# mihikamd/DP-GSAT

Hardware: AMD Instinct MI355X
Metric: million edges/s (attn+sample+aggregate fwd+bwd) (higher is better)
Workload: dtype f32

## Files before the change

dp_gsat_amd/csrc/common.h:

```cpp
#pragma once
#include <cstring>
#include <cstdint>
#include <cstdio>
#include <cstdarg>
#include <hip/hip_runtime.h>

#include "../../include/gsat_hip.h"

namespace gsat {

void set_error(const char* fmt, ...);
const char* get_error();

#define GSAT_CHECK_HIP(expr)                                                                  \
    do {                                                                                      \
        hipError_t _e = (expr);                                                               \
        if (_e != hipSuccess) {                                                               \
            gsat::set_error("%s:%d: %s -> %s", __FILE__, __LINE__, #expr, hipGetErrorString(_e)); \
            return GSAT_ERR_HIP;                                                              \
        }                                                                                     \
    } while (0)

#define GSAT_REQUIRE(cond, code, ...)                                                         \
    do {                                                                                      \
        if (!(cond)) {                                                                        \
            gsat::set_error(__VA_ARGS__);                                                     \
            return (code);                                                                    \
        }                                                                                     \
    } while (0)

#define GSAT_LAUNCH_CHECK() GSAT_CHECK_HIP(hipGetLastError())

static inline int64_t ceil_div(int64_t a, int64_t b) { return (a + b - 1) / b; }

hipError_t zero_async(void* p, size_t bytes, hipStream_t stream);
static inline size_t align_up(size_t a, size_t b) { return (a + b - 1) / b * b; }

struct Arena {
    char* base;
    size_t cap, off;
    Arena(void* p, size_t bytes) : base(static_cast<char*>(p)), cap(bytes), off(0) {}
    template <class T> T* take(size_t n) {
        size_t b = align_up(n * sizeof(T), 256);
        if (base == nullptr || off + b > cap) { off += b; return nullptr; }
        T* r = reinterpret_cast<T*>(base + off);
        off += b;
        return r;
    }
    bool ok() const { return base != nullptr && off <= cap; }
};

struct SlabJob { const float* ws; int nslab; size_t slab; int M, N; int64_t ldc; int accumulate; float* out; };
int gemm_f32(hipStream_t stream, bool a_t, bool b_t, int64_t M, int64_t N, int64_t K, const float* A, int64_t lda, const float* B,
             int64_t ldb, float* C, int64_t ldc, const float* bias, bool accumulate, float* ws, size_t ws_floats, bool allow_split = false,
             SlabJob* defer = nullptr);
int slab_reduce_jobs(hipStream_t stream, const SlabJob* jobs, int n);
size_t gemm_workspace_floats(int64_t M, int64_t N, int64_t K, bool reduce_rows);
struct WgradPlan { int eligible, S, rows; size_t ws_floats; };
WgradPlan wgrad_plan(int64_t Mo, int64_t No, int64_t K);
size_t gemm_wgrad_workspace_floats(int64_t Mo, int64_t No, int64_t K);
int gemm_wgrad(hipStream_t stream, int64_t Mo, int64_t No, int64_t K, const float* A, int64_t lda, const float* B, int64_t ldb, float* C,
               int64_t ldc, bool accumulate, float* ws, size_t ws_floats, SlabJob* defer = nullptr);

int aggr_sum_fwd_impl(hipStream_t stream, const float* x, const float* self_rows, const float* att, const float* edge_emb,
                      const int32_t* rowptr, const int32_t* col, const int32_t* eid, int64_t N, int64_t E, int64_t H, float self_coef,
                      float* out, const int32_t* chunk_ptr, float* partial);

#ifdef __HIPCC__
constexpr int WAVE = 64;

template <int CTRL> __device__ __forceinline__ float dpp_add(float v) {
    const int t = __builtin_amdgcn_update_dpp(0, __builtin_bit_cast(int, v), CTRL, 0xF, 0xF, true);
    return v + __builtin_bit_cast(float, t);
}

template <int WIDTH> __device__ __forceinline__ float group_sum(float v) {
    if constexpr ((WIDTH & (WIDTH - 1)) == 0) {
        if constexpr (WIDTH >= 2) v = dpp_add<0xB1>(v);
        if constexpr (WIDTH >= 4) v = dpp_add<0x4E>(v);
        if constexpr (WIDTH >= 8) v = dpp_add<0x141>(v);
        if constexpr (WIDTH >= 16) v = dpp_add<0x140>(v);
        if constexpr (WIDTH >= 32) v += __builtin_bit_cast(float, __builtin_amdgcn_ds_swizzle(__builtin_bit_cast(int, v), 0x401F));
        if constexpr (WIDTH >= 64) v += __shfl_xor(v, 32, 64);
    } else {
        const int l = (int)(threadIdx.x & 63) % WIDTH;
#pragma unroll
        for (int o = 16; o > 0; o >>= 1) {
            const float t = __shfl_down(v, o, 64);
            if (l + o < WIDTH) v += t;
        }
    }
    return v;
}

template <int LPR, int BLOCK> struct LaneGroups {
    static constexpr int GPW = 64 / LPR, GPB = (BLOCK / 64) * GPW;
    int grp, lane;
    __device__ __forceinline__ LaneGroups() {
        const int wl = threadIdx.x & 63, sub = wl / LPR;
        lane = wl % LPR;
        grp = sub < GPW ? (int)(threadIdx.x >> 6) * GPW + sub : -1;
    }
};

__device__ __forceinline__ float4 ld4(const float* p) { return *reinterpret_cast<const float4*>(p); }
__device__ __forceinline__ void st4(float* p, float4 v) { *reinterpret_cast<float4*>(p) = v; }
__device__ __forceinline__ void st4_nt(float* p, float4 v) {
    typedef float v4f __attribute__((ext_vector_type(4)));
    v4f t = {v.x, v.y, v.z, v.w};
    __builtin_nontemporal_store(t, reinterpret_cast<v4f*>(p));
}
__device__ __forceinline__ float4 ld4_off(const float* base, uint32_t byte_off) {
    return *reinterpret_cast<const float4*>(reinterpret_cast<const char*>(base) + byte_off);
}
__device__ __forceinline__ void st4_off(float* base, uint32_t byte_off, float4 v) {
    *reinterpret_cast<float4*>(reinterpret_cast<char*>(base) + byte_off) = v;
}
__device__ __forceinline__ void st4_lds(float4* p, float4 v) {
    typedef float v4f __attribute__((ext_vector_type(4)));
    v4f t = {v.x, v.y, v.z, v.w};
    *(__attribute__((address_space(3))) v4f*)p = t;
}
__device__ __forceinline__ void st1_lds(float* p, float v) { *(__attribute__((address_space(3))) float*)p = v; }
__device__ __forceinline__ float4 f4zero() { return make_float4(0.f, 0.f, 0.f, 0.f); }
__device__ __forceinline__ float4 f4fma(float a, float4 x, float4 acc) {
    acc.x = fmaf(a, x.x, acc.x); acc.y = fmaf(a, x.y, acc.y);
    acc.z = fmaf(a, x.z, acc.z); acc.w = fmaf(a, x.w, acc.w);
    return acc;
}
__device__ __forceinline__ float f4dot(float4 a, float4 b) {
    return fmaf(a.x, b.x, fmaf(a.y, b.y, fmaf(a.z, b.z, a.w * b.w)));
}

__device__ __forceinline__ uint4 philox4x32(uint64_t seed, uint32_t c0, uint32_t c1, uint32_t c2, uint32_t c3) {
    uint32_t k0 = (uint32_t)seed, k1 = (uint32_t)(seed >> 32);
#pragma unroll
    for (int r = 0; r < 10; ++r) {
        uint64_t p0 = (uint64_t)0xD2511F53u * c0;
        uint64_t p1 = (uint64_t)0xCD9E8D57u * c2;
        uint32_t n0 = (uint32_t)(p1 >> 32) ^ c1 ^ k0;
        uint32_t n1 = (uint32_t)p1;
        uint32_t n2 = (uint32_t)(p0 >> 32) ^ c3 ^ k1;
        uint32_t n3 = (uint32_t)p0;
        c0 = n0; c1 = n1; c2 = n2; c3 = n3;
        k0 += 0x9E3779B9u; k1 += 0xBB67AE85u;
    }
    return make_uint4(c0, c1, c2, c3);
}

__device__ __forceinline__ float philox_noise_u(uint64_t seed, int row) {
    const uint4 r = philox4x32(seed, (uint32_t)row, 0u, 4u, 0x5A17u);
    return ((float)(r.x >> 9) + 0.5f) * (1.0f / 8388608.0f);
}

struct SeedRef {
    uint64_t value;
    const uint64_t* dev;
    __device__ __forceinline__ uint64_t get() const { return dev ? *dev : value; }
};

__device__ __forceinline__ float4 philox_keep4(uint64_t seed, int layer, int row, int c, float p) {
    uint4 r = philox4x32(seed, (uint32_t)row, (uint32_t)(c >> 2), (uint32_t)layer, 0x5A17u);
    const float k = 1.0f / 16777216.0f;
    return make_float4((float)(r.x >> 8) * k >= p ? 1.f : 0.f, (float)(r.y >> 8) * k >= p ? 1.f : 0.f,
                       (float)(r.z >> 8) * k >= p ? 1.f : 0.f, (float)(r.w >> 8) * k >= p ? 1.f : 0.f);
}
#endif

}
```

dp_gsat_amd/csrc/pna.hip:

```cpp
#include "common.h"
#include "pna_math.h"

namespace gsat {

constexpr int PNA_BLOCK = 128;
constexpr int SC_AMP = GSAT_SCALE_AMPLIFICATION, SC_ATT = GSAT_SCALE_ATTENUATION, SC_LIN = GSAT_SCALE_LINEAR, SC_INVLIN = GSAT_SCALE_INVERSE_LINEAR;

struct PnaCfg {
    int A, S;
    int aggr[8];
    int scal[8];
    float avg_lin, avg_log;
};

__device__ __forceinline__ int pna_xcd_remap(int b, int nb) {
    int q = nb >> 3, r = nb & 7, x = b & 7, i = b >> 3;
    return (x < r ? x * (q + 1) : r * (q + 1) + (x - r) * q) + i;
}

__device__ __forceinline__ float scaler_factor(int s, float deg, float avg_lin, float avg_log) {
    switch (s) {
        case SC_AMP: return logf(deg + 1.f) / avg_log;
        case SC_ATT: return deg == 0.f ? 1.f : avg_log / logf(deg + 1.f);
        case SC_LIN: return deg / avg_lin;
// ... 420 lines not shown
                        aj.add(m);
                        if (HAS_EE) {
                            float4 me = f4scale(w[u], ev[u]);
                            if (me.x < ae.mn.x) emin.x = kk; if (me.y < ae.mn.y) emin.y = kk; if (me.z < ae.mn.z) emin.z = kk; if (me.w < ae.mn.w) emin.w = kk;
                            if (me.x > ae.mx.x) emax.x = kk; if (me.y > ae.mx.y) emax.y = kk; if (me.z > ae.mx.z) emax.z = kk; if (me.w > ae.mx.w) emax.w = kk;
                            ae.add(me);
                        }
                    }
                }
            }
        }
        const Acc4 ai = self_stats(xi, sa, sa2, amin, amax);
        float t1 = 0.f, t2 = 0.f, tmn = 0.f, tmx = 0.f;
        float4 Pi = f4zero(), Qi = f4zero(), Pj = f4zero(), Qj = f4zero(), Pe = f4zero(), Qe = f4zero();
        float4 gmn_i = f4zero(), gmx_i = f4zero(), gmn_j = f4zero(), gmx_j = f4zero(), gmn_e = f4zero(), gmx_e = f4zero();
        if (on) {
            const float n = fmaxf(cnt, 1.f), inv_n = 1.f / n;
            const float* drow = dout + (size_t)row * out_stride + c;
            if (staged) asm volatile("s_waitcnt vmcnt(0)" ::: "memory");
#define GSAT_FOLD(ACC, PART, P, Q, GMN, GMX)                                                                           \
            {                                                                                                          \
                const float4 mean = f4scale(inv_n, ACC.s);                                                             \
                float4 var = make_float4(ACC.q.x * inv_n - mean.x * mean.x, ACC.q.y * inv_n - mean.y * mean.y,         \
                                         ACC.q.z * inv_n - mean.z * mean.z, ACC.q.w * inv_n - mean.w * mean.w);        \
                const float4 hs = make_float4(var.x > 0.f ? 0.5f / sqrtf(var.x + 1e-5f) : 0.f, var.y > 0.f ? 0.5f / sqrtf(var.y + 1e-5f) : 0.f, \
                                              var.z > 0.f ? 0.5f / sqrtf(var.z + 1e-5f) : 0.f, var.w > 0.f ? 0.5f / sqrtf(var.w + 1e-5f) : 0.f); \
                float4 p0 = f4zero(), gv = f4zero();                                                                   \
                if (NAGG) {                                                                                            \
                    p0 = f4scale(inv_n, stage[0 * parts + (PART)][threadIdx.x]);                                       \
                    if (NAGG == 5) { const float4 vsum = stage[4 * parts + (PART)][threadIdx.x];                       \
                                     p0 = make_float4(p0.x + vsum.x, p0.y + vsum.y, p0.z + vsum.z, p0.w + vsum.w); }   \
                    GMN = stage[1 * parts + (PART)][threadIdx.x];                                                      \
                    GMX = stage[2 * parts + (PART)][threadIdx.x];                                                      \
                    const float4 vs = stage[3 * parts + (PART)][threadIdx.x];                                          \
                    gv = make_float4(vs.x * hs.x, vs.y * hs.y, vs.z * hs.z, vs.w * hs.w);                              \
                } else                                                                                                 \
                for (int s = 0; s < cfg.S; ++s) {                                                                      \
                    const float f = scaler_factor(cfg.scal[s], cnt, cfg.avg_lin, cfg.avg_log);                         \
                    for (int a = 0; a < cfg.A; ++a) {                                                                  \
                        const int sg_ = (s * cfg.A + a) * parts + (PART);                                              \
                        const float4 v = f4scale(f, staged ? stage[sg_][threadIdx.x] : ld4(drow + (size_t)sg_ * H));   \
                        switch (cfg.aggr[a]) {                                                                         \
                            case AGG_SUM: p0.x += v.x; p0.y += v.y; p0.z += v.z; p0.w += v.w; break;                   \
                            case AGG_MEAN: p0 = f4fma(inv_n, v, p0); break;                                            \
                            case AGG_MIN: GMN.x += v.x; GMN.y += v.y; GMN.z += v.z; GMN.w += v.w; break;               \
                            case AGG_MAX: GMX.x += v.x; GMX.y += v.y; GMX.z += v.z; GMX.w += v.w; break;               \
                            case AGG_VAR: gv.x += v.x; gv.y += v.y; gv.z += v.z; gv.w += v.w; break;                   \
                            default: gv.x = fmaf(v.x, hs.x, gv.x); gv.y = fmaf(v.y, hs.y, gv.y);                       \
                                     gv.z = fmaf(v.z, hs.z, gv.z); gv.w = fmaf(v.w, hs.w, gv.w); break;                \
                        }                                                                                              \
                    }                                                                                                  \
                }                                                                                                      \
                Q = f4scale(2.f * inv_n, gv);                                                                          \
                P = make_float4(p0.x - mean.x * Q.x, p0.y - mean.y * Q.y, p0.z - mean.z * Q.z, p0.w - mean.w * Q.w);   \
            }
            GSAT_FOLD(ai, 0, Pi, Qi, gmn_i, gmx_i)
            {
#define GSAT_SELF(C)                                                                                                   \
            {                                                                                                          \
                const float xc = xi.C;                                                                                 \
                const float wlo = xc > 0.f ? amin : (xc < 0.f ? amax : wfirst), whi = xc > 0.f ? amax : (xc < 0.f ? amin : wfirst); \
                dxi.C = Pi.C * sa + Qi.C * xc * sa2 + gmn_i.C * wlo + gmx_i.C * whi;                                   \
                t1 = fmaf(Pi.C, xc, t1);                                                                               \
                t2 = fmaf(Qi.C * xc, xc, t2);                                                                          \
                tmn += xc > 0.f ? gmn_i.C * xc : (xc < 0.f ? gmx_i.C * xc : 0.f);                                      \
                tmx += xc > 0.f ? gmx_i.C * xc : (xc < 0.f ? gmn_i.C * xc : 0.f);                                      \
            }
            float4 dxi;
            GSAT_SELF(x) GSAT_SELF(y) GSAT_SELF(z) GSAT_SELF(w)
#undef GSAT_SELF
            st4(dx_self + (size_t)row * H + c, dxi);
            }
            GSAT_FOLD(aj, 1, Pj, Qj, gmn_j, gmx_j)
            if (HAS_EE) { GSAT_FOLD(ae, 2, Pe, Qe, gmn_e, gmx_e) }
#undef GSAT_FOLD
        }
        if (LONG) {
            float* r = partial + (size_t)chunk_ptr[row] * rec;
            if (on) {
                st4(r + c, Pj); st4(r + H + c, Qj); st4(r + 2 * H + c, gmn_j); st4(r + 3 * H + c, gmx_j);
                st4i(r + 4 * H + c, jmin); st4i(r + 5 * H + c, jmax);
                if (HAS_EE) {
                    float* re = r + 6 * H;
                    st4(re + c, Pe); st4(re + H + c, Qe); st4(re + 2 * H + c, gmn_e); st4(re + 3 * H + c, gmx_e);
                    st4i(re + 4 * H + c, emin); st4i(re + 5 * H + c, emax);
                }
            }
            const float s1 = group_sum<LPR>(t1), s2 = group_sum<LPR>(t2), smn = group_sum<LPR>(tmn), smx = group_sum<LPR>(tmx);
            if (lane == 0) {
                st4(r + (size_t)6 * GP * H, make_float4(s1, s2, smn, smx));
                st4(r + (size_t)6 * GP * H + 4, make_float4(__int_as_float(kmin_a), __int_as_float(kmax_a), 0.f, 0.f));
            }
            continue;
        }
        for (int kb = beg; kb < end; kb += 4) {
            const int nb = min(4, end - kb);
            int j4[4], e4[4];
            float w4[4];
            float4 x4[4], ee4[4];
            if (end - beg <= 4) {
#pragma unroll
                for (int u = 0; u < 4; ++u) { j4[u] = lj[u]; e4[u] = le[u]; w4[u] = lw[u]; }
            } else {
#pragma unroll
                for (int u = 0; u < 4; ++u) {
                    j4[u] = u < nb ? col[kb + u] : 0;
                    e4[u] = u < nb ? eid[kb + u] : 0;
                }
#pragma unroll
                for (int u = 0; u < 4; ++u) w4[u] = (u < nb && att) ? att[e4[u]] : 1.f;
            }
#pragma unroll
            for (int u = 0; u < 4; ++u) {
                x4[u] = (u < nb && on) ? ld4(x + (size_t)j4[u] * H + c) : f4zero();
                if (HAS_EE) ee4[u] = (u < nb && on) ? ld4(edge_emb + (size_t)e4[u] * H + c) : f4zero();
            }
#pragma unroll
            for (int u = 0; u < 4; ++u) {
                if (u >= nb) continue;
                const int k = kb + u, e = e4[u];
                const float w = w4[u];
                const float4 xj = x4[u];
                float da = 0.f;
                if (on) {
                    float4 dm;
                    dm.x = fmaf(Qj.x, w * xj.x, Pj.x) + (k == jmin.x ? gmn_j.x : 0.f) + (k == jmax.x ? gmx_j.x : 0.f);
                    dm.y = fmaf(Qj.y, w * xj.y, Pj.y) + (k == jmin.y ? gmn_j.y : 0.f) + (k == jmax.y ? gmx_j.y : 0.f);
                    dm.z = fmaf(Qj.z, w * xj.z, Pj.z) + (k == jmin.z ? gmn_j.z : 0.f) + (k == jmax.z ? gmx_j.z : 0.f);
                    dm.w = fmaf(Qj.w, w * xj.w, Pj.w) + (k == jmin.w ? gmn_j.w : 0.f) + (k == jmax.w ? gmx_j.w : 0.f);
                    st4(dmsg + (size_t)k * H + c, f4scale(w, dm));
                    da += f4dot(dm, xj);
                    da += t1 + w * t2 + (k == kmin_a ? tmn : 0.f) + (k == kmax_a ? tmx : 0.f);
                    if (HAS_EE) {
                        const float4 ee = ee4[u];
                        float4 de;
                        de.x = fmaf(Qe.x, w * ee.x, Pe.x) + (k == emin.x ? gmn_e.x : 0.f) + (k == emax.x ? gmx_e.x : 0.f);
                        de.y = fmaf(Qe.y, w * ee.y, Pe.y) + (k == emin.y ? gmn_e.y : 0.f) + (k == emax.y ? gmx_e.y : 0.f);
                        de.z = fmaf(Qe.z, w * ee.z, Pe.z) + (k == emin.z ? gmn_e.z : 0.f) + (k == emax.z ? gmx_e.z : 0.f);
                        de.w = fmaf(Qe.w, w * ee.w, Pe.w) + (k == emin.w ? gmn_e.w : 0.f) + (k == emax.w ? gmx_e.w : 0.f);
                        if (dedge) st4(dedge + (size_t)e * H + c, f4scale(w, de));
                        da += f4dot(de, ee);
                    }
                }
                if (datt) {
                    da = group_sum<LPR>(da);
                    if (lane == 0) datt[e] = c0 ? datt[e] + da : da;
                }
            }
        }
    }
}

constexpr int TILE_BLOCK = 512;

__global__ void k_pna_tiles(const int32_t* __restrict__ node_ptr, const int32_t* __restrict__ node_seg, const int32_t* __restrict__ rowptr,
                            const int32_t* __restrict__ rowptr_src, int N, int TN, int slack, int T, int4* __restrict__ desc,
                            int32_t* __restrict__ spill_count) {
    const int t = blockIdx.x * blockDim.x + threadIdx.x;
    if (t == 0 && spill_count) *spill_count = 0;
    if (t > T) return;
    const int64_t p = (int64_t)t * TN;
    int start = N;
    if (t < T && p < N) {
        start = (int)p;
        if (node_seg) {
            const int g0 = node_ptr[node_seg[p]];
            start = min((int)p, max(g0, (int)p - slack));
        }
    }
    desc[t] = make_int4(start, rowptr[start], rowptr_src[start], 0);
}

template <int LPR, int NAGG, bool NATT>
__global__ __launch_bounds__(TILE_BLOCK, 4) void k_pna_bwd_tile(
    const float* __restrict__ x, const float* __restrict__ att, const float* __restrict__ dout, const int32_t* __restrict__ rowptr,
    const int32_t* __restrict__ col, const int32_t* __restrict__ eid, const int4* __restrict__ desc,
    const int32_t* __restrict__ rowptr_src, const int32_t* __restrict__ slot_map, int H, int TE, int RCAP, float* dx,
    float* __restrict__ dmsg, float* datt, float* __restrict__ dw, const float* __restrict__ dx_add, int datt_acc) {
    constexpr int GPB = LaneGroups<LPR, TILE_BLOCK>::GPB;
    constexpr int RPW = 64 / LPR;
    constexpr int NSEG = NAGG * 2;
    extern __shared__ float4 smem4[];
    float4* erow = smem4;
    int* s_col = reinterpret_cast<int*>(erow + (size_t)TE * LPR);
    int* s_eid = s_col + TE;
    float* s_w = reinterpret_cast<float*>(s_eid);
    float* s_att = reinterpret_cast<float*>(s_eid + TE);
    int* s_slot = reinterpret_cast<int*>(s_att + TE);
    int* s_rp = s_slot + TE;
    int* s_rps = s_rp + RCAP + 1;
    float* s_na = reinterpret_cast<float*>(s_rps + RCAP + 1);
    float* s_dna = s_na + RCAP + 1;
    const int tid = threadIdx.x, wave = tid >> 6;
    const LaneGroups<LPR, TILE_BLOCK> lg;
    const int grp = lg.grp < 0 ? GPB : lg.grp;
    const int lane = lg.lane, c = lane * 4;
    const bool on = c < H && lg.grp >= 0;
    const int t = pna_xcd_remap(blockIdx.x, gridDim.x);
    const int4 d0 = desc[t], d1 = desc[t + 1];
    const int n0 = d0.x, n1 = d1.x;
    if (n1 <= n0) return;
    const int nr = n1 - n0;
    const int k0 = d0.y, ne = min(d1.y - k0, TE);
    const int s0 = d0.z, ns = d1.z - s0, nsl = min(ns, TE);
    float4 dcur[NSEG];
    float4 xi_cur = f4zero();
    const uint32_t hb = (uint32_t)H * 4u, gb = NSEG * hb, cb = (uint32_t)c * 4u;
    const float* gwin = dout + (size_t)n0 * NSEG * H;
    const float* xwin = x + (size_t)n0 * H;
    float* dxwin = dx + (size_t)n0 * H;
    float* mwin = dmsg + (size_t)k0 * H;
    int r = lg.grp >= 0 ? grp : nr;
#pragma unroll
    for (int sg = 0; sg < NSEG; ++sg) dcur[sg] = f4zero();
    if (r < nr && on) {
#pragma unroll
        for (int sg = 0; sg < NSEG; ++sg) dcur[sg] = ld4_off(gwin, r * gb + sg * hb + cb);
        xi_cur = ld4_off(xwin, r * hb + cb);
    }
    for (int i = tid; i <= nr; i += TILE_BLOCK) {
        s_rp[i] = rowptr[n0 + i] - k0;
        s_rps[i] = rowptr_src[n0 + i] - s0;
        if (NATT) { s_na[i] = att[min(n0 + i, n1 - 1)]; s_dna[i] = 0.f; }
    }
    for (int i = tid; i < ne; i += TILE_BLOCK) {
        s_col[i] = col[k0 + i];
        if (!NATT) s_eid[i] = eid[k0 + i];
    }
    for (int i = tid; i < nsl; i += TILE_BLOCK) s_slot[i] = slot_map[s0 + i] - k0;
    __syncthreads();
    for (int base = 0; base < ne; base += GPB) {
        const int i = base + grp;
        if (i < ne && on)
            __builtin_amdgcn_global_load_lds((const __attribute__((address_space(1))) void*)(x + (size_t)s_col[i] * H + c),
                                             (__attribute__((address_space(3))) void*)(erow + (size_t)(base + wave * RPW) * LPR), 16, 0, 0);
    }
    for (int i = tid; i < ne; i += TILE_BLOCK) {
        if (NATT) {
            s_att[i] = att[s_col[i]];
        } else {
            s_att[i] = att ? att[s_eid[i]] : 1.f;
        }
    }
    asm volatile("s_waitcnt vmcnt(0)" ::: "memory");
    __syncthreads();
    float4 dx_keep = f4zero();
    for (; r < nr; r += GPB) {
        const int nr_ = r + GPB;
        const int beg = s_rp[r], end = s_rp[r + 1];
        const float na_row = NATT ? s_na[r] : 0.f;
        const float cnt = (float)(end - beg);
        float sa = 0.f, sa2 = 0.f, amin = INFINITY, amax = -INFINITY;
        int kmin_a = beg, kmax_a = beg;
        Acc4 aj;
        aj.init();
        int4 jmin = make_int4(beg, beg, beg, beg), jmax = jmin;
        float wfirst = 1.f;
        const int mid = min(end, max(beg, ne));
        auto stats = [&](int k, float w, float4 xv) {
            if (k == beg) wfirst = w;
            sa += w; sa2 = fmaf(w, w, sa2);
            if (w < amin) { amin = w; kmin_a = k; }
            if (w > amax) { amax = w; kmax_a = k; }
            const float4 m = f4scale(w, xv);
#define GSAT_TARG(C)                                                                                                       \
            if (m.C < aj.mn.C) { jmin.C = k; aj.mn.C = m.C; }                                                              \
            if (m.C > aj.mx.C) { jmax.C = k; aj.mx.C = m.C; }
            GSAT_TARG(x) GSAT_TARG(y) GSAT_TARG(z) GSAT_TARG(w)
#undef GSAT_TARG
            aj.s.x += m.x; aj.s.y += m.y; aj.s.z += m.z; aj.s.w += m.w;
            aj.q.x = fmaf(m.x, m.x, aj.q.x); aj.q.y = fmaf(m.y, m.y, aj.q.y); aj.q.z = fmaf(m.z, m.z, aj.q.z); aj.q.w = fmaf(m.w, m.w, aj.q.w);
        };
        for (int k = beg; k < mid; ++k)
            stats(k, NATT ? s_att[k] * na_row : s_att[k], on ? erow[(size_t)k * LPR + lane] : f4zero());
        for (int k = mid; k < end; ++k)
            stats(k, NATT ? att[col[k0 + k]] * na_row : (att ? att[eid[k0 + k]] : 1.f), on ? ld4(x + (size_t)col[k0 + k] * H + c) : f4zero());
        const float4 xi = xi_cur;
        const Acc4 ai = self_stats(xi, sa, sa2, amin, amax);
        const float n = fmaxf(cnt, 1.f), inv_n = 1.f / n;
        float t1 = 0.f, t2 = 0.f, tmn = 0.f, tmx = 0.f;
        float4 Pi, Qi, Pj, Qj, gmn_i, gmx_i, gmn_j, gmx_j;
#define GSAT_TFOLD(ACC, PART, P, Q, GMN, GMX)                                                                              \
        {                                                                                                                  \
            const float4 mean = f4scale(inv_n, ACC.s);                                                                     \
            const float4 var = make_float4(ACC.q.x * inv_n - mean.x * mean.x, ACC.q.y * inv_n - mean.y * mean.y,           \
                                           ACC.q.z * inv_n - mean.z * mean.z, ACC.q.w * inv_n - mean.w * mean.w);          \
            const float4 hs = make_float4(var.x > 0.f ? 0.5f * __builtin_amdgcn_rsqf(var.x + 1e-5f) : 0.f,                 \
                                          var.y > 0.f ? 0.5f * __builtin_amdgcn_rsqf(var.y + 1e-5f) : 0.f,                 \
                                          var.z > 0.f ? 0.5f * __builtin_amdgcn_rsqf(var.z + 1e-5f) : 0.f,                 \
                                          var.w > 0.f ? 0.5f * __builtin_amdgcn_rsqf(var.w + 1e-5f) : 0.f);                \
            float4 p0 = f4scale(inv_n, dcur[0 * 2 + (PART)]);                                                              \
            if (NAGG == 5) { const float4 vsum = dcur[(NAGG == 5 ? 4 : 0) * 2 + (PART)];                                   \
                             p0 = make_float4(p0.x + vsum.x, p0.y + vsum.y, p0.z + vsum.z, p0.w + vsum.w); }               \
            GMN = dcur[1 * 2 + (PART)];                                                                                    \
            GMX = dcur[2 * 2 + (PART)];                                                                                    \
            const float4 vs = dcur[3 * 2 + (PART)];                                                                        \
            const float4 gv = make_float4(vs.x * hs.x, vs.y * hs.y, vs.z * hs.z, vs.w * hs.w);                             \
            Q = f4scale(2.f * inv_n, gv);                                                                                  \
            P = make_float4(p0.x - mean.x * Q.x, p0.y - mean.y * Q.y, p0.z - mean.z * Q.z, p0.w - mean.w * Q.w);           \
        }
        GSAT_TFOLD(ai, 0, Pi, Qi, gmn_i, gmx_i)
        if (on) {
            float4 dxi;
#define GSAT_TSELF(C)                                                                                                      \
            {                                                                                                              \
                const float xc = xi.C;                                                                                     \
                const float wlo = xc > 0.f ? amin : (xc < 0.f ? amax : wfirst), whi = xc > 0.f ? amax : (xc < 0.f ? amin : wfirst); \
                dxi.C = Pi.C * sa + Qi.C * xc * sa2 + gmn_i.C * wlo + gmx_i.C * whi;                                       \
                t1 = fmaf(Pi.C, xc, t1);                                                                                   \
                t2 = fmaf(Qi.C * xc, xc, t2);                                                                              \
                tmn += xc > 0.f ? gmn_i.C * xc : (xc < 0.f ? gmx_i.C * xc : 0.f);                                          \
                tmx += xc > 0.f ? gmx_i.C * xc : (xc < 0.f ? gmn_i.C * xc : 0.f);                                          \
            }
            GSAT_TSELF(x) GSAT_TSELF(y) GSAT_TSELF(z) GSAT_TSELF(w)
#undef GSAT_TSELF
            if (end == beg) dxi = f4zero();
            if (nr_ < nr) st4_off(dxwin, r * hb + cb, dxi); else dx_keep = dxi;
        }
        GSAT_TFOLD(aj, 1, Pj, Qj, gmn_j, gmx_j)
#undef GSAT_TFOLD
        if (nr_ < nr && on) {
#pragma unroll
            for (int sg = 0; sg < NSEG; ++sg) dcur[sg] = ld4_off(gwin, nr_ * gb + sg * hb + cb);
            xi_cur = ld4_off(xwin, nr_ * hb + cb);
        }
        float dna_acc = 0.f;
        auto grad = [&](int k, float w, float a_src, int j, int e, float4 xj, bool lds) {
            const bool in_lds = lds && j >= n0 && j < n1;
            float da = 0.f;
            if (on) {
                float4 dm;
                dm.x = fmaf(Qj.x, w * xj.x, Pj.x) + (k == jmin.x ? gmn_j.x : 0.f) + (k == jmax.x ? gmx_j.x : 0.f);
                dm.y = fmaf(Qj.y, w * xj.y, Pj.y) + (k == jmin.y ? gmn_j.y : 0.f) + (k == jmax.y ? gmx_j.y : 0.f);
                dm.z = fmaf(Qj.z, w * xj.z, Pj.z) + (k == jmin.z ? gmn_j.z : 0.f) + (k == jmax.z ? gmx_j.z : 0.f);
                dm.w = fmaf(Qj.w, w * xj.w, Pj.w) + (k == jmin.w ? gmn_j.w : 0.f) + (k == jmax.w ? gmx_j.w : 0.f);
                const float4 o = f4scale(w, dm);
                if (in_lds) st4_lds(erow + (size_t)k * LPR + lane, o);
                else if (lds) st4_off(mwin, k * hb + cb, o);
                else st4(dmsg + (size_t)(k0 + k) * H + c, o);
                da = f4dot(dm, xj) + t1 + w * t2 + (k == kmin_a ? tmn : 0.f) + (k == kmax_a ? tmx : 0.f);
            }
            if (datt) {
                da = group_sum<LPR>(da);
                if (NATT) {
                    if (lane == 0) {
                        dna_acc = fmaf(da, a_src, dna_acc);
                        const float share = da * na_row;
                        if (in_lds) st1_lds(s_w + k, share); else dw[k0 + k] = share;
                    }
                } else if (lane == 0) datt[e] = da;
            }
        };
        for (int k = beg; k < mid; ++k) {
            const float a = s_att[k];
            grad(k, NATT ? a * na_row : a, a, s_col[k], NATT ? 0 : s_eid[k], on ? erow[(size_t)k * LPR + lane] : f4zero(), true);
        }
        for (int k = mid; k < end; ++k) {
            const int j = col[k0 + k], e = NATT ? 0 : eid[k0 + k];
            const float a = NATT ? att[j] : (att ? att[e] : 1.f);
            grad(k, NATT ? a * na_row : a, a, j, e, on ? ld4(x + (size_t)j * H + c) : f4zero(), false);
        }
        if (NATT && datt && lane == 0) s_dna[r] = dna_acc;
    }
    __syncthreads();
    const float* awin = dx_add ? dx_add + (size_t)n0 * H : nullptr;
    for (int j = lg.grp >= 0 ? grp : nr; j < nr; j += GPB) {
        if (!on) continue;
        const int sb = s_rps[j], se = s_rps[j + 1];
        float4 acc = j + GPB < nr ? ld4_off(dxwin, j * hb + cb) : dx_keep;
        const float dprev = (NATT && datt && datt_acc && lane == 0) ? datt[n0 + j] : 0.f;
        if (awin) {
            const float4 ra = ld4_off(awin, j * hb + cb);
            acc.x += ra.x; acc.y += ra.y; acc.z += ra.z; acc.w += ra.w;
        }
        float sw = 0.f;
        for (int s_ = sb; s_ < se; ++s_) {
            const int kl = s_ < nsl ? s_slot[s_] : slot_map[s0 + s_] - k0;
            if (kl >= 0 && kl < ne) {
                const float4 v = erow[(size_t)kl * LPR + lane];
                acc.x += v.x; acc.y += v.y; acc.z += v.z; acc.w += v.w;
                if (NATT && datt) sw += s_w[kl];
            }
        }
        st4_off(dxwin, j * hb + cb, acc);
        if (NATT && datt && lane == 0) datt[n0 + j] = (s_dna[j] + sw) + dprev;
    }
}

__global__ void k_pna_spill_rows(const int4* __restrict__ desc, int TN, int TE, const int32_t* __restrict__ rowptr_src,
                                 const int32_t* __restrict__ slot_map, int num_rows, int32_t* __restrict__ spill_rows,
                                 int32_t* __restrict__ spill_count) {
    const int j = blockIdx.x * blockDim.x + threadIdx.x;
    if (j >= num_rows) return;
    const int sb = rowptr_src[j], se = rowptr_src[j + 1];
    if (sb == se) return;
    int t = j / TN;
    if (j >= desc[t + 1].x) ++t;
    const int k0 = desc[t].y, ne = min(desc[t + 1].y - k0, TE);
    bool flag = false;
    for (int s_ = sb; s_ < se && !flag; ++s_) {
        const int k = slot_map[s_];
        flag = k < k0 || k >= k0 + ne;
    }
    if (flag) {
        const int idx = atomicAdd(spill_count, 1);
        if (idx < num_rows) spill_rows[idx] = j;
    }
}

template <int LPR>
__global__ __launch_bounds__(256) void k_pna_bwd_spill(const float* __restrict__ dmsg, const int4* __restrict__ desc, int TN, int TE,
                                                       const int32_t* __restrict__ rowptr_src, const int32_t* __restrict__ slot_map,
                                                       const int32_t* __restrict__ spill_rows, const int32_t* __restrict__ spill_count,
                                                       int num_rows, int H, float* __restrict__ dx, const float* __restrict__ dw,
                                                       float* __restrict__ dna) {
    const LaneGroups<LPR, 256> lg;
    constexpr int GPB = LaneGroups<LPR, 256>::GPB;
    const int lane = lg.lane, c = lane * 4;
    const int count = min(*spill_count, num_rows);
    if (lg.grp < 0) return;
    for (int i = blockIdx.x * GPB + lg.grp; i < count; i += gridDim.x * GPB) {
        const int j = spill_rows[i];
        const int sb = rowptr_src[j], se = rowptr_src[j + 1];
        int t = j / TN;
        if (j >= desc[t + 1].x) ++t;
        const int k0 = desc[t].y, ne = min(desc[t + 1].y - k0, TE);
        if (c >= H) continue;
        float4 acc = ld4(dx + (size_t)j * H + c);
        float sw = 0.f;
        for (int s_ = sb; s_ < se; ++s_) {
            const int k = slot_map[s_];
            if (k >= k0 && k < k0 + ne) continue;
            const float4 v = ld4(dmsg + (size_t)k * H + c);
            acc.x += v.x; acc.y += v.y; acc.z += v.z; acc.w += v.w;
            if (dna) sw += dw[k];
        }
        st4(dx + (size_t)j * H + c, acc);
        if (dna && lane == 0) dna[j] += sw;
    }
}

static inline int pna_lpr(int64_t H) {
    if (H <= 0 || H % 4 != 0 || H > 256) return 0;
    int64_t q = H / 4;
    return q <= 4 ? 4 : q <= 8 ? 8 : q <= 16 ? 16 : q <= 20 ? 20 : q <= 32 ? 32 : 64;
}

constexpr int PNA_CHUNK = 256;
static inline bool pna_width_ok(int64_t H) { return H > 0 && H % 4 == 0 && H <= 512; }

static inline void pna_grid(int64_t N, int lpr, int* nb, int* rpg) {
    const int gpb = (PNA_BLOCK / 64) * (64 / lpr);
    int64_t b = ceil_div(N, gpb);
    if (b > 256 * 64) b = 256 * 64;
    if (b < 1) b = 1;
    *nb = (int)b;
    *rpg = (int)std::max<int64_t>(1, ceil_div(N, b * gpb));
}

static inline int fixed_aggregators(const PnaCfg& cfg) {
    if (cfg.S != 1 || cfg.scal[0] != 0 || (cfg.A != 4 && cfg.A != 5)) return 0;
    if (cfg.aggr[0] != AGG_MEAN || cfg.aggr[1] != AGG_MIN || cfg.aggr[2] != AGG_MAX || cfg.aggr[3] != GSAT_AGG_STD) return 0;
    if (cfg.A == 5 && cfg.aggr[4] != AGG_SUM) return 0;
    return cfg.A;
}

static int make_cfg(const int32_t* aggr, int A, const int32_t* scal, int S, float avg_lin, float avg_log, PnaCfg* cfg) {
    GSAT_REQUIRE(aggr && scal && A >= 1 && A <= 8 && S >= 1 && S <= 8, GSAT_ERR_ARG, "pna: need 1..8 aggregators and scalers");
    cfg->A = A; cfg->S = S; cfg->avg_lin = avg_lin; cfg->avg_log = avg_log;
    for (int i = 0; i < 8; ++i) { cfg->aggr[i] = 0; cfg->scal[i] = 0; }
    for (int i = 0; i < A; ++i) {
        GSAT_REQUIRE(aggr[i] >= 0 && aggr[i] <= 5, GSAT_ERR_ARG, "pna: unknown aggregator code %d", aggr[i]);
        cfg->aggr[i] = aggr[i];
    }
    for (int i = 0; i < S; ++i) {
        GSAT_REQUIRE(scal[i] >= 0 && scal[i] <= 4, GSAT_ERR_ARG, "pna: unknown scaler code %d", scal[i]);
        cfg->scal[i] = scal[i];
    }
    return GSAT_OK;
}

template <int L, int NA, bool NATT>
static hipError_t pna_tile_allow_lds(size_t lds) {
    static size_t allowed = 0;
    if (lds <= allowed) return hipSuccess;
    hipError_t e = hipFuncSetAttribute((const void*)k_pna_bwd_tile<L, NA, NATT>, hipFuncAttributeMaxDynamicSharedMemorySize, (int)lds);
    if (e == hipSuccess) allowed = lds;
    return e;
}

static size_t pna_tile_lds_bytes(int lpr, int edges_cap, int rows_cap) {
    return (size_t)edges_cap * ((size_t)lpr * 16 + 16) + (size_t)(rows_cap + 1) * 16;
}

}

using namespace gsat;

#define GSAT_LPR_DISPATCH(lpr, CALL) \
    switch (lpr) { case 4: CALL(4); break; case 8: CALL(8); break; case 16: CALL(16); break; case 20: CALL(20); break; case 32: CALL(32); break; default: CALL(64); break; }

extern "C" {

static int pna_fwd_impl(const char* who, const float* x, const float* att, const float* edge_emb, const int32_t* rowptr, const int32_t* col,
                        const int32_t* eid, int64_t N, int64_t E, int64_t H, const int32_t* aggregators, int A, const int32_t* scalers, int S,
                        float avg_deg_lin, float avg_deg_log, float* out, const int32_t* chunk_ptr, float* partial, hipStream_t stream,
                        float* scal_out = nullptr) {
    GSAT_REQUIRE(N >= 0 && N < (1ll << 31), GSAT_ERR_ARG, "%s: bad N", who);
    PnaCfg cfg;
    int rc = make_cfg(aggregators, A, scalers, S, avg_deg_lin, avg_deg_log, &cfg);
    if (rc) return rc;
    if (N == 0) return GSAT_OK;
    GSAT_REQUIRE(pna_width_ok(H), GSAT_ERR_UNSUPPORTED, "%s: H=%lld must be a multiple of 4 and <= 512", who, (long long)H);
    GSAT_REQUIRE(x && rowptr && out, GSAT_ERR_ARG, "%s: null pointer", who);
    GSAT_REQUIRE(chunk_ptr == nullptr || partial != nullptr, GSAT_ERR_ARG, "%s: chunk_ptr needs the record workspace", who);
    if (E <= CH) chunk_ptr = nullptr;
    const int nagg = fixed_aggregators(cfg);
    GSAT_REQUIRE(!scal_out || (nagg && !edge_emb && !chunk_ptr), GSAT_ERR_UNSUPPORTED,
                 "%s: the compact output needs (mean,min,max,std[,sum]) with the identity scaler, no edge features, no hub chunks", who);
    for (int c0 = 0; c0 < (int)H; c0 += PNA_CHUNK) {
        const int Hc = std::min<int>(PNA_CHUNK, (int)H - c0);
        const int lpr = pna_lpr(Hc);
        int nb, rpg;
        pna_grid(N, lpr, &nb, &rpg);
        const int gpb = (PNA_BLOCK / 64) * (64 / lpr);
        const int cb = chunk_ptr ? (int)std::min<int64_t>(ceil_div(pna_max_chunks(E), gpb), 256 * 16) : 0;
#define GO(L, EE, NA)                                                                                                                       \
    do {                                                                                                                                    \
        k_pna_fwd<L, EE, NA, false><<<nb, PNA_BLOCK, 0, stream>>>(x, att, edge_emb, rowptr, col, eid, (int)N, (int)H, cfg, out, rpg, c0, Hc, chunk_ptr, partial, scal_out); \
        if (cb) k_pna_fwd<L, EE, NA, true><<<cb, PNA_BLOCK, 0, stream>>>(x, att, edge_emb, rowptr, col, eid, (int)N, (int)H, cfg, out, rpg, c0, Hc, chunk_ptr, partial, scal_out); \
    } while (0)
#define CALL(L)                                                                                                              \
    do {                                                                                                                     \
        if (edge_emb) {                                                                                                      \
            if (cb) k_pna_chunk_stats<L, true><<<cb, PNA_BLOCK, 0, stream>>>(x, att, edge_emb, rowptr, col, eid, (int)N, (int)H, chunk_ptr, partial, c0, Hc); \
            if (nagg == 4) GO(L, true, 4); else if (nagg == 5) GO(L, true, 5); else GO(L, true, 0);                          \
        } else {                                                                                                             \
            if (cb) k_pna_chunk_stats<L, false><<<cb, PNA_BLOCK, 0, stream>>>(x, att, edge_emb, rowptr, col, eid, (int)N, (int)H, chunk_ptr, partial, c0, Hc); \
// ... 213 lines not shown
```

Measured before the change: 130.5.

## Prefetch scatter-phase rows before barrier and keep last rows in registers

In the PNA backward tile kernel, the final one to three dx rows per lane group now stay in registers instead of being stored and reloaded. The first five dx, dx_add and datt values for the scatter phase are prefetched before the __syncthreads so their latency overlaps the barrier. Gradient window loads switch to nontemporal loads. This costs more registers and adds select logic, which may lower occupancy.

```diff
diff --git a/dp_gsat_amd/csrc/common.h b/dp_gsat_amd/csrc/common.h
--- a/dp_gsat_amd/csrc/common.h
+++ b/dp_gsat_amd/csrc/common.h
@@ -113,6 +113,11 @@
 __device__ __forceinline__ float4 ld4_off(const float* base, uint32_t byte_off) {
     return *reinterpret_cast<const float4*>(reinterpret_cast<const char*>(base) + byte_off);
 }
+__device__ __forceinline__ float4 ld4_off_nt(const float* base, uint32_t byte_off) {
+    typedef float v4f __attribute__((ext_vector_type(4)));
+    const v4f t = __builtin_nontemporal_load(reinterpret_cast<const v4f*>(reinterpret_cast<const char*>(base) + byte_off));
+    return make_float4(t.x, t.y, t.z, t.w);
+}
 __device__ __forceinline__ void st4_off(float* base, uint32_t byte_off, float4 v) {
     *reinterpret_cast<float4*>(reinterpret_cast<char*>(base) + byte_off) = v;
 }
@@ -123,6 +128,10 @@
 }
 __device__ __forceinline__ void st1_lds(float* p, float v) { *(__attribute__((address_space(3))) float*)p = v; }
 __device__ __forceinline__ float4 f4zero() { return make_float4(0.f, 0.f, 0.f, 0.f); }
+__device__ __forceinline__ float f1sel(bool c, float a, float b) { return c ? a : b; }
+__device__ __forceinline__ float4 f4sel(bool c, float4 a, float4 b) {
+    return make_float4(f1sel(c, a.x, b.x), f1sel(c, a.y, b.y), f1sel(c, a.z, b.z), f1sel(c, a.w, b.w));
+}
 __device__ __forceinline__ float4 f4fma(float a, float4 x, float4 acc) {
     acc.x = fmaf(a, x.x, acc.x); acc.y = fmaf(a, x.y, acc.y);
     acc.z = fmaf(a, x.z, acc.z); acc.w = fmaf(a, x.w, acc.w);
diff --git a/dp_gsat_amd/csrc/pna.hip b/dp_gsat_amd/csrc/pna.hip
--- a/dp_gsat_amd/csrc/pna.hip
+++ b/dp_gsat_amd/csrc/pna.hip
@@ -596,6 +596,8 @@
 }
 
 constexpr int TILE_BLOCK = 512;
+constexpr int TILE_PREFETCH = 5;
+constexpr int pna_tile_keep(int lpr, int nagg, bool natt) { return (lpr == 20 && nagg == 5 && natt) ? 2 : 3; }
 
 __global__ void k_pna_tiles(const int32_t* __restrict__ node_ptr, const int32_t* __restrict__ node_seg, const int32_t* __restrict__ rowptr,
                             const int32_t* __restrict__ rowptr_src, int N, int TN, int slack, int T, int4* __restrict__ desc,
@@ -659,7 +661,7 @@
     for (int sg = 0; sg < NSEG; ++sg) dcur[sg] = f4zero();
     if (r < nr && on) {
 #pragma unroll
-        for (int sg = 0; sg < NSEG; ++sg) dcur[sg] = ld4_off(gwin, r * gb + sg * hb + cb);
+        for (int sg = 0; sg < NSEG; ++sg) dcur[sg] = ld4_off_nt(gwin, r * gb + sg * hb + cb);
         xi_cur = ld4_off(xwin, r * hb + cb);
     }
     for (int i = tid; i <= nr; i += TILE_BLOCK) {
@@ -688,7 +690,9 @@
     }
     asm volatile("s_waitcnt vmcnt(0)" ::: "memory");
     __syncthreads();
-    float4 dx_keep = f4zero();
+    constexpr int K = pna_tile_keep(LPR, NAGG, NATT);
+    static_assert(K >= 1 && K <= 3 && K < TILE_PREFETCH, "k_pna_bwd_tile keeps one to three rows");
+    float4 keep0 = f4zero(), keep1 = f4zero(), keep2 = f4zero();
     for (; r < nr; r += GPB) {
         const int nr_ = r + GPB;
         const int beg = s_rp[r], end = s_rp[r + 1];
@@ -759,13 +763,16 @@
             GSAT_TSELF(x) GSAT_TSELF(y) GSAT_TSELF(z) GSAT_TSELF(w)
 #undef GSAT_TSELF
             if (end == beg) dxi = f4zero();
-            if (nr_ < nr) st4_off(dxwin, r * hb + cb, dxi); else dx_keep = dxi;
+            if (r + K * GPB < nr) st4_off(dxwin, r * hb + cb, dxi);
+            if (K > 2) keep2 = keep1;
+            if (K > 1) keep1 = keep0;
+            keep0 = dxi;
         }
         GSAT_TFOLD(aj, 1, Pj, Qj, gmn_j, gmx_j)
 #undef GSAT_TFOLD
         if (nr_ < nr && on) {
 #pragma unroll
-            for (int sg = 0; sg < NSEG; ++sg) dcur[sg] = ld4_off(gwin, nr_ * gb + sg * hb + cb);
+            for (int sg = 0; sg < NSEG; ++sg) dcur[sg] = ld4_off_nt(gwin, nr_ * gb + sg * hb + cb);
             xi_cur = ld4_off(xwin, nr_ * hb + cb);
         }
         float dna_acc = 0.f;
@@ -806,17 +813,42 @@
         }
         if (NATT && datt && lane == 0) s_dna[r] = dna_acc;
     }
+    constexpr int PF = TILE_PREFETCH;
+    const float* awin = dx_add ? dx_add + (size_t)n0 * H : nullptr;
+    const bool want_prev = NATT && datt && datt_acc;
+    const int jg = lg.grp >= 0 ? grp : nr;
+    const int cnt = jg < nr ? (nr - 1 - jg) / GPB + 1 : 0;
+    float4 pdx[PF], padd[PF];
+    float pprev[PF];
+#pragma unroll
+    for (int i = 0; i < PF; ++i) {
+        pdx[i] = f4zero();
+        padd[i] = f4zero();
+        pprev[i] = 0.f;
+    }
+    if (on) {
+#pragma unroll
+        for (int i = 0; i < PF; ++i) pdx[i] = ld4_off(dxwin, (i + K < cnt ? jg + i * GPB : nr - 1) * hb + cb);
+        if (awin) {
+#pragma unroll
+            for (int i = 0; i < PF; ++i) padd[i] = ld4_off(awin, min(jg + i * GPB, nr - 1) * hb + cb);
+        }
+        if (want_prev) {
+#pragma unroll
+            for (int i = 0; i < PF; ++i) pprev[i] = datt[n0 + min(jg + i * GPB, nr - 1)];
+        }
+    }
     __syncthreads();
-    const float* awin = dx_add ? dx_add + (size_t)n0 * H : nullptr;
-    for (int j = lg.grp >= 0 ? grp : nr; j < nr; j += GPB) {
-        if (!on) continue;
+    if (!on) return;
+    auto kept = [&](int rem) {
+        float4 v = keep0;
+        if (K > 1) v = f4sel(rem == 1, keep1, v);
+        if (K > 2) v = f4sel(rem == 2, keep2, v);
+        return v;
+    };
+    auto sums = [&](int j, float4 acc, float4 ra, float dprev) {
         const int sb = s_rps[j], se = s_rps[j + 1];
-        float4 acc = j + GPB < nr ? ld4_off(dxwin, j * hb + cb) : dx_keep;
-        const float dprev = (NATT && datt && datt_acc && lane == 0) ? datt[n0 + j] : 0.f;
-        if (awin) {
-            const float4 ra = ld4_off(awin, j * hb + cb);
-            acc.x += ra.x; acc.y += ra.y; acc.z += ra.z; acc.w += ra.w;
-        }
+        if (awin) { acc.x += ra.x; acc.y += ra.y; acc.z += ra.z; acc.w += ra.w; }
         float sw = 0.f;
         for (int s_ = sb; s_ < se; ++s_) {
             const int kl = s_ < nsl ? s_slot[s_] : slot_map[s0 + s_] - k0;
@@ -828,6 +860,23 @@
         }
         st4_off(dxwin, j * hb + cb, acc);
         if (NATT && datt && lane == 0) datt[n0 + j] = (s_dna[j] + sw) + dprev;
+    };
+    auto prefetched = [&](auto I) {
+        constexpr int i = decltype(I)::value;
+        const int j = jg + i * GPB, rem = cnt - 1 - i;
+        if (j >= nr) return false;
+        sums(j, f4sel(rem >= K, pdx[i], kept(rem)), padd[i], (want_prev && lane == 0) ? pprev[i] : 0.f);
+        return true;
+    };
+    static_assert(PF == 5, "one call per prefetched row");
+    using std::integral_constant;
+    if (!(prefetched(integral_constant<int, 0>{}) && prefetched(integral_constant<int, 1>{}) && prefetched(integral_constant<int, 2>{}) &&
+          prefetched(integral_constant<int, 3>{}) && prefetched(integral_constant<int, 4>{})))
+        return;
+    for (int j = jg + PF * GPB, rem = cnt - 1 - PF; j < nr; j += GPB, --rem) {
+        const float4 acc = rem >= K ? ld4_off(dxwin, j * hb + cb) : kept(rem);
+        const float4 ra = awin ? ld4_off(awin, j * hb + cb) : f4zero();
+        sums(j, acc, ra, (want_prev && lane == 0) ? datt[n0 + j] : 0.f);
     }
 }
 
```

Result: faster. 133.4 (median of 6 runs) (+2.2%).
